# levs57/halo2-liam-eagen-msm

Hardware: AMD Instinct MI355X
Metric: BN254 G1 MSM scalar-point-pairs/s (higher is better)
Workload: dtype u32 limbs (256-bit Montgomery integers)

## Files before the change

### halo2_liam_eagen_msm_amd/api.py

```python
from __future__ import annotations

import ctypes
import math
from typing import List, Optional, Sequence, Tuple

import numpy as np

from . import _lib
from ._lib import BN254_G1, GRUMPKIN

ORDER = {
    BN254_G1: 0x30644E72E131A029B85045B68181585D2833E84879B9709143E1F593F0000001,
    GRUMPKIN: 0x30644E72E131A029B85045B68181585D97816A916871CA8D3C208C16D87CFD47,
}
CURVE_IDS = {"bn254_g1": BN254_G1, "grumpkin": GRUMPKIN}


class LemsmError(RuntimeError):
    def __init__(self, status: int, msg: str):
        super().__init__(f"lemsm status {status}: {msg}")
        self.status = status


class LengthMismatch(LemsmError, AssertionError):
# ... 671 lines not shown
        self._check(self.lib.lemsm_device_gen_walk(self.h, _curve_id(curve), _ptr(q), n, buf.ptr))
        return buf

    def debug_montmul(self, curve, a, b) -> np.ndarray:
        a = _limbs(a, 4); b = _limbs(b, 4)
        out = np.zeros_like(a)
        self._check(self.lib.lemsm_debug_montmul(self.h, _curve_id(curve), _ptr(a), _ptr(b), _ptr(out), a.shape[0]))
        return out

    def debug_fieldop(self, curve, op: int, a, b) -> np.ndarray:
        a = _limbs(a, 4); b = _limbs(b, 4)
        out = np.zeros_like(a)
        self._check(self.lib.lemsm_debug_fieldop(self.h, _curve_id(curve), op, _ptr(a), _ptr(b), _ptr(out), a.shape[0]))
        return out

    def debug_pointop(self, curve, op: int, acc_xyzz, q) -> np.ndarray:
        acc = _limbs(acc_xyzz, 16)
        q = _limbs(q, 16 if op == 1 else 8)
        out = np.zeros_like(acc)
        self._check(self.lib.lemsm_debug_pointop(self.h, _curve_id(curve), op, _ptr(acc), _ptr(q), _ptr(out), acc.shape[0]))
        return out

    F29_OPS = ("mul", "sqr", "mul2", "mul_addhi", "sqr_addhi", "add", "sub", "neg", "cneg", "wnorm", "canon", "reduce_small",
               "mul32", "from_abi", "div32", "is_zero_mod", "limbs_zero", "hi_term", "pp_is_zero")
    X29_OPS = ("madd", "madd_abi", "add", "dbl_affine", "dbl", "scale", "unscale", "add4_mem")

    def debug_field29_raw(self, curve, op, a, b=None, c=None, d=None) -> np.ndarray:
        opi = self.F29_OPS.index(op) if isinstance(op, str) else int(op)
        a = np.ascontiguousarray(a, np.int32).reshape(-1, 9)
        ops = [a] + [np.zeros_like(a) if x is None else np.ascontiguousarray(x, np.int32).reshape(-1, 9) for x in (b, c, d)]
        if any(x.shape != a.shape for x in ops):
            raise ValueError("field29_raw operands must all be n x 9 int32")
        out = np.zeros((a.shape[0], 10), np.int32)
        self._check(self.lib.lemsm_debug_field29_raw(self.h, _curve_id(curve), opi, *[_ptr(x) for x in ops], _ptr(out), a.shape[0]))
        return out

    def debug_xyzz29_raw(self, curve, op, acc, q=None) -> np.ndarray:
        opi = self.X29_OPS.index(op) if isinstance(op, str) else int(op)
        acc = np.ascontiguousarray(acc, np.int32).reshape(-1, 37)
        q = np.zeros_like(acc) if q is None else np.ascontiguousarray(q, np.int32).reshape(-1, 37)
        if q.shape != acc.shape:
            raise ValueError("xyzz29_raw records must both be n x 37 int32")
        out = np.zeros_like(acc)
        self._check(self.lib.lemsm_debug_xyzz29_raw(self.h, _curve_id(curve), opi, _ptr(acc), _ptr(q), _ptr(out), acc.shape[0]))
        return out


# ... 387 lines not shown
```

### halo2_liam_eagen_msm_amd/csrc/field29.cuh

```cuda
#pragma once
#include <hip/hip_runtime.h>
#include <stdint.h>

namespace lemsm {

typedef int32_t i32;
typedef int64_t i64;
typedef uint32_t u32;
typedef uint64_t u64;

struct Fq29Params {
  static constexpr i32 N[9] = {0x187cfd47, 0x010460b6, 0x1c72a34f, 0x02d522d0, 0x1585d978, 0x02db40c0, 0x00a6e141, 0x0e5c2634, 0x0030644e};
  static constexpr u32 NINV = 0x04866389u;
  static constexpr i32 ONE[9] = {0x157ccc21, 0x141c2758, 0x185230d3, 0x014c0419, 0x0aa36fb9, 0x1d4240ce, 0x11d54c07, 0x052ac7a8, 0x000dc836};
  static constexpr i32 C266[9] = {0x13349ca1, 0x1a5d84a8, 0x0a3e5cac, 0x100249e0, 0x12b951e8, 0x0e92d304, 0x14cb95b3, 0x041b9d3d, 0x00058003};
  static constexpr i32 C256[9] = {0x058f0d9d, 0x1aea1c6e, 0x11c2cf74, 0x11d651eb, 0x1462c0a7, 0x11b7bc3c, 0x1cbd99ba, 0x183340fb, 0x000e0a77};
};
struct Fr29Params {
  static constexpr i32 N[9] = {0x10000001, 0x1f0fac9f, 0x0e5c2450, 0x07d090f3, 0x1585d283, 0x02db40c0, 0x00a6e141, 0x0e5c2634, 0x0030644e};
  static constexpr u32 NINV = 0x0fffffffu;
  static constexpr i32 ONE[9] = {0x0fffff57, 0x1ea70ab4, 0x052c068b, 0x17504f49, 0x0aa8075b, 0x1d4240ce, 0x11d54c07, 0x052ac7a8, 0x000dc836};
  static constexpr i32 C266[9] = {0x0fffead7, 0x1d5444f4, 0x04438aa5, 0x03b4d096, 0x134c84da, 0x0e92d304, 0x14cb95b3, 0x041b9d3d, 0x00058003};
  static constexpr i32 C256[9] = {0x0ffffffb, 0x04b1a0e2, 0x18334a6b, 0x18ed2b3e, 0x1462e36f, 0x11b7bc3c, 0x1cbd99ba, 0x183340fb, 0x000e0a77};
};
// ... 11 lines not shown
  static __device__ __forceinline__ void set_one(fe& r) {
#pragma unroll
    for (int i = 0; i < 9; i++) r.l[i] = P::ONE[i];
  }
  static __device__ __forceinline__ bool limbs_zero(const fe& a) {
    i32 o = 0;
#pragma unroll
    for (int i = 0; i < 9; i++) o |= a.l[i];
    return o == 0;
  }
  static __device__ __forceinline__ void sub(fe& r, const fe& a, const fe& b) {
#pragma unroll
    for (int i = 0; i < 9; i++) r.l[i] = a.l[i] - b.l[i];
  }
  static __device__ __forceinline__ void add(fe& r, const fe& a, const fe& b) {
#pragma unroll
    for (int i = 0; i < 9; i++) r.l[i] = a.l[i] + b.l[i];
  }
  static __device__ __forceinline__ void neg(fe& r, const fe& a) {
#pragma unroll
    for (int i = 0; i < 9; i++) r.l[i] = -a.l[i];
  }
  static __device__ __forceinline__ void cneg(fe& r, const fe& a, bool flag) {
    i32 s = flag ? -1 : 0;
#pragma unroll
    for (int i = 0; i < 9; i++) r.l[i] = (a.l[i] ^ s) - s;
  }
  static __device__ __forceinline__ void wnorm(fe& a) {
    i32 c = 0;
#pragma unroll
    for (int i = 0; i < 8; i++) {
      i32 v = a.l[i] + c;
      a.l[i] = v & MASK;
      c = v >> 29;
    }
    a.l[8] += c;
  }

#include "field29_gen.inc"

  static __device__ __forceinline__ void canon(fe& a) {
    i32 c = 0;
#pragma unroll
    for (int i = 0; i < 9; i++) {
      i32 n8 = (i32)((((u32)P::N[i] << 3) & (u32)MASK) | (i ? ((u32)P::N[i - 1] >> 26) : 0u));
      i32 v = a.l[i] + n8 + c;
      if (i < 8) { a.l[i] = v & MASK; c = v >> 29; } else a.l[i] = v;
    }
#pragma unroll
// ... 45 lines not shown
    unpack(r, w);
  }
  static __device__ __forceinline__ void store(void* p, const fe& a) {
    fe t = a; canon(t);
    u32 w[8]; pack(w, t);
    uint4* q = reinterpret_cast<uint4*>(p);
    q[0] = make_uint4(w[0], w[1], w[2], w[3]);
    q[1] = make_uint4(w[4], w[5], w[6], w[7]);
  }
  static __device__ __forceinline__ void from_abi(fe& r, const fe& a) {
    fe c;
#pragma unroll
    for (int i = 0; i < 9; i++) c.l[i] = P::C266[i];
    mul(r, a, c);
  }
  static __device__ __forceinline__ void div32(fe& r, const fe& a) {
    fe c;
#pragma unroll
    for (int i = 0; i < 9; i++) c.l[i] = P::C256[i];
    mul(r, a, c);
  }
  static __device__ __forceinline__ void mul32(fe& r, const fe& a) {
    const float inv = 32.0f / (float)P::N[8];
    i32 q = (i32)((float)a.l[8] * inv);
    i64 t = 0;
#pragma unroll
    for (int i = 0; i < 9; i++) {
      t += (i64)a.l[i] * 32 - (i64)q * P::N[i];
      if (i < 8) { r.l[i] = (i32)t & MASK; t >>= 29; }
      else r.l[i] = (i32)t;
    }
  }
  static __device__ __forceinline__ void reduce_small(fe& r, const fe& a) {
    const float inv = 1.0f / (float)P::N[8];
    i32 q = (i32)((float)a.l[8] * inv);
    i64 t = 0;
#pragma unroll
    for (int i = 0; i < 9; i++) {
      t += (i64)a.l[i] - (i64)q * P::N[i];
      if (i < 8) { r.l[i] = (i32)t & MASK; t >>= 29; }
      else r.l[i] = (i32)t;
    }
  }
  static __device__ __forceinline__ void set_c266(fe& r) {
#pragma unroll
    for (int i = 0; i < 9; i++) r.l[i] = P::C266[i];
  }
};

}
```

### halo2_liam_eagen_msm_amd/csrc/field29_gen.inc

```
  static __device__ __forceinline__ void mul(fe& r, const fe& a, const fe& b) {
    i64 acc = 0;
    i32 m0, m1, m2, m3, m4, m5, m6, m7, m8;
    acc += (i64)a.l[0] * (i64)b.l[0];
    m0 = (i32)(((u32)acc * P::NINV) & (u32)MASK);
    acc += (i64)m0 * (i64)P::N[0];
    acc >>= 29;
    asm("v_mad_i64_i32 %0, vcc, %1, %2, %0\n\t"
        "v_mad_i64_i32 %0, vcc, %3, %4, %0\n\t"
        "v_mad_i64_i32 %0, vcc, %5, %6, %0\n\t" : "+v"(acc) : "v"(a.l[0]), "v"(b.l[1]), "v"(a.l[1]), "v"(b.l[0]), "v"(m0), "s"(P::N[1]) : "vcc");
    m1 = (i32)(((u32)acc * P::NINV) & (u32)MASK);
    acc += (i64)m1 * (i64)P::N[0];
    acc >>= 29;
    asm("v_mad_i64_i32 %0, vcc, %1, %2, %0\n\t"
        "v_mad_i64_i32 %0, vcc, %3, %4, %0\n\t"
        "v_mad_i64_i32 %0, vcc, %5, %6, %0\n\t"
        "v_mad_i64_i32 %0, vcc, %7, %8, %0\n\t"
        "v_mad_i64_i32 %0, vcc, %9, %10, %0\n\t" : "+v"(acc) : "v"(a.l[0]), "v"(b.l[2]), "v"(a.l[1]), "v"(b.l[1]), "v"(a.l[2]), "v"(b.l[0]), "v"(m0), "s"(P::N[2]), "v"(m1), "s"(P::N[1]) : "vcc");
    m2 = (i32)(((u32)acc * P::NINV) & (u32)MASK);
    acc += (i64)m2 * (i64)P::N[0];
    acc >>= 29;
    asm("v_mad_i64_i32 %0, vcc, %1, %2, %0\n\t"
        "v_mad_i64_i32 %0, vcc, %3, %4, %0\n\t"
        "v_mad_i64_i32 %0, vcc, %5, %6, %0\n\t"
        "v_mad_i64_i32 %0, vcc, %7, %8, %0\n\t"
// ... 986 lines not shown
    acc >>= 29;
    asm("v_mad_i64_i32 %0, vcc, %1, %2, %0\n\t"
        "v_mad_i64_i32 %0, vcc, %3, %4, %0\n\t"
        "v_mad_i64_i32 %0, vcc, %5, %6, %0\n\t"
        "v_mad_i64_i32 %0, vcc, %7, %8, %0\n\t"
        "v_mad_i64_i32 %0, vcc, %9, %10, %0\n\t" : "+v"(acc) : "v"(a2_6), "v"(a.l[8]), "v"(a.l[7]), "v"(a.l[7]), "v"(m6), "s"(P::N[8]), "v"(m7), "s"(P::N[7]), "v"(m8), "s"(P::N[6]) : "vcc");
    acc += (i64)hi.l[5];
    r.l[5] = (i32)((u32)acc & (u32)MASK);
    acc >>= 29;
    asm("v_mad_i64_i32 %0, vcc, %1, %2, %0\n\t"
        "v_mad_i64_i32 %0, vcc, %3, %4, %0\n\t"
        "v_mad_i64_i32 %0, vcc, %5, %6, %0\n\t" : "+v"(acc) : "v"(a2_7), "v"(a.l[8]), "v"(m7), "s"(P::N[8]), "v"(m8), "s"(P::N[7]) : "vcc");
    acc += (i64)hi.l[6];
    r.l[6] = (i32)((u32)acc & (u32)MASK);
    acc >>= 29;
    asm("v_mad_i64_i32 %0, vcc, %1, %2, %0\n\t"
        "v_mad_i64_i32 %0, vcc, %3, %4, %0\n\t" : "+v"(acc) : "v"(a.l[8]), "v"(a.l[8]), "v"(m8), "s"(P::N[8]) : "vcc");
    acc += (i64)hi.l[7];
    r.l[7] = (i32)((u32)acc & (u32)MASK);
    acc >>= 29;
    acc += (i64)hi.l[8];
    r.l[8] = (i32)acc;
  }
```

### halo2_liam_eagen_msm_amd/csrc/kernels_ec.cuh

```cuda
#pragma once
#include "plan.h"
#include "xyzz.cuh"
#include "xyzz29.cuh"

namespace lemsm {

static const u32 KEY_NONE = 0xffffffffu;

enum { META_M = 0, META_TILES = 1, META_WORDS = 4, META_CLOCK = 8  };

template <class G, int WPS ,
          bool ABI = false ,
          bool RING = false >
__global__ __launch_bounds__(256, WPS) void k_accum1(GroupPlan pl, const u32* __restrict__ sorted,
                                                const u32* __restrict__ bucket_start, u32* __restrict__ meta,
                                                const uint4* __restrict__ points, char* __restrict__ bucket_sum,
                                                u32* __restrict__ rec_key, char* __restrict__ rec_pt) {
  typedef typename G::F_ F;
  typedef typename F::fe fe;
  const u32 t = blockIdx.x * 256 + threadIdx.x;
  if (t >= pl.nthr1) return;
  const u32 M = meta[META_M];
  const bool stamp = blockIdx.x == (gridDim.x >> 1) && threadIdx.x == 0;
  if (stamp) {
// ... 31 lines not shown
  };

  __shared__ u32 ering[RING ? 4 : 1][2][4][64][RING ? 4 : 1];
  const u32 wv = threadIdx.x >> 6, lane = threadIdx.x & 63u;
  auto ring_fill = [&](u32 blk) {
#pragma unroll
    for (int k = 0; k < 4; k++)
      __builtin_amdgcn_global_load_lds((const __attribute__((address_space(1))) void*)(sorted + start + 16u * blk + 4u * k),
                                       (__attribute__((address_space(3))) void*)&ering[wv][blk & 1u][k][0][0], 16, 0, 0);
  };
  auto ring_read = [&](u32 rel) -> u32 { return ering[wv][(rel >> 4) & 1u][(rel >> 2) & 3u][lane][rel & 3u]; };
  u32 e_next;
  if constexpr (RING) {
    ring_fill(0);
    if (pl.L1 > 16) ring_fill(1);
    asm volatile("s_waitcnt vmcnt(0)" ::: "memory");
    e_next = ring_read(0);
  } else {
    e_next = sorted[start];
  }
  uint4 nx0, nx1, ny0, ny1;
  { const uint4* p = points + (size_t)(e_next & 0xffffffu) * 4; nx0 = p[0]; nx1 = p[1]; ny0 = p[2]; ny1 = p[3]; }

  for (u32 i = start; i < end; i++) {
    u32 e = e_next; fe px, py;
    F::from_words(px, nx0, nx1); F::from_words(py, ny0, ny1);
    if (i >= kend) {
      flush(i);
      key++; kend = kend2; kend2 = kend3;
      while (i >= kend) { key++; kend = kend2; kend2 = bucket_start[min(key + 2u, nkeys)]; }
      kbeg = i; seg_begin = i;
      G::set_identity(acc); empty = true;
    }
    if (i + 1 < end) {
      if constexpr (RING) {
        const u32 rel1 = i + 1 - start;
        if ((rel1 & 15u) == 0) asm volatile("s_waitcnt vmcnt(0)" ::: "memory");
        e_next = ring_read(rel1);
        if ((rel1 & 15u) == 0 && rel1 + 16u < pl.L1) ring_fill((rel1 >> 4) + 1u);
      } else {
        e_next = sorted[i + 1];
      }
      const uint4* p = points + (size_t)(e_next & 0xffffffu) * 4;
      nx0 = p[0]; nx1 = p[1]; ny0 = p[2]; ny1 = p[3];
    }
    kend3 = bucket_start[min(key + 3u, nkeys)];
    if (!G::aff_is_identity(px, py)) {
      F::cneg(py, py, (e >> 31) != 0);
      if (ABI) G::madd_abi(acc, px, py, empty); else G::madd(acc, px, py, empty);
    }
  }
  flush(end);
  if (stamp) {
    u64* ck = reinterpret_cast<u64*>(meta + META_CLOCK);
    ck[2] = __builtin_amdgcn_s_memtime(); ck[3] = __builtin_amdgcn_s_memrealtime();
  }
  rec_key[t] = (seg_begin == kbeg && end != kend) ? key : KEY_NONE;
}

enum { MQ_S = 0, MQ_M = 1, MQ_L = 2, MQ_F = 3, MQ_P = 4, MQ_WORDS = 16  };
static const u32 MQ_DST_BUCKET = 0xffffffffu;

template <class G>
__device__ __forceinline__ void merge_load_piece(typename G::pt& q, const char* __restrict__ rec_pt, u32 t, bool first_slot, u32 scaled) {
  G::load(q, rec_pt + (size_t)(2u * t + (first_slot ? 0u : 1u)) * G::PT_BYTES);
// ... 344 lines not shown
```

### halo2_liam_eagen_msm_amd/csrc/lemsm.hip

```cpp
#include <hip/hip_runtime.h>
#include <math.h>
#include <stdio.h>
#include <stdlib.h>
#include <string.h>

#include <algorithm>
#include <cmath>
#include <map>
#include <string>
#include <vector>

#include "../../include/lemsm.h"
#include "hostmath.hpp"
#include "hostpool.hpp"
#include "hosttail.hpp"
#include <memory>
#include "kernels.cuh"
#include "rccl_dyn.hpp"
#include "roctx_dyn.hpp"
#include "divisor.cuh"
#include "regfn_eval.cuh"
#include "regfn_logderiv.cuh"
#include "rhs.cuh"
#include <rocprim/rocprim.hpp>
// ... 1352 lines not shown
  raw_ld<F29>(x, a + 9 * (size_t)i); raw_ld<F29>(y, b + 9 * (size_t)i); raw_ld<F29>(z, c + 9 * (size_t)i); raw_ld<F29>(w, d + 9 * (size_t)i);
  int32_t pred = 0;
  r = x;
  switch (op) {
    case 0: F29::mul(r, x, y); break;
    case 1: F29::sqr(r, x); break;
    case 2: F29::mul2(r, x, y, z, w); break;
    case 3: F29::mul_addhi(r, x, y, z); break;
    case 4: F29::sqr_addhi(r, x, z); break;
    case 5: F29::add(r, x, y); break;
    case 6: F29::sub(r, x, y); break;
    case 7: F29::neg(r, x); break;
    case 8: F29::cneg(r, x, y.l[0] != 0); break;
    case 9: F29::wnorm(r); break;
    case 10: F29::canon(r); break;
    case 11: F29::reduce_small(r, x); break;
    case 12: F29::mul32(r, x); break;
    case 13: F29::from_abi(r, x); break;
    case 14: F29::div32(r, x); break;
    case 15: pred = F29::is_zero_mod(x) ? 1 : 0; break;
    case 16: pred = F29::limbs_zero(x) ? 1 : 0; break;
    case 17: G29::hi_term(r, x, y); break;
    case 18: pred = G29::pp_is_zero(x) ? 1 : 0; break;
    default: break;
  }
  int32_t* o = out + 10 * (size_t)i;
  raw_st<F29>(o, r);
  o[9] = pred;
}

template <class G29>
__device__ __forceinline__ void raw_ld_pt(typename G29::pt& p, const int32_t* s) {
  typedef typename G29::F_ F29;
  raw_ld<F29>(p.x, s); raw_ld<F29>(p.y, s + 9); raw_ld<F29>(p.zz, s + 18); raw_ld<F29>(p.zzz, s + 27);
}
template <class G29>
__device__ __forceinline__ void raw_st_pt(int32_t* s, const typename G29::pt& p) {
  typedef typename G29::F_ F29;
  raw_st<F29>(s, p.x); raw_st<F29>(s + 9, p.y); raw_st<F29>(s + 18, p.zz); raw_st<F29>(s + 27, p.zzz);
}
template <class G29>
__global__ void k_dbg_xyzz29_raw(int op, const int32_t* __restrict__ acc_in, const int32_t* __restrict__ q_in, int32_t* __restrict__ out, u32 n) {
  u32 i = blockIdx.x * blockDim.x + threadIdx.x;
  if (i >= n) return;
  const int32_t* ap = acc_in + (size_t)i * 37;
  const int32_t* qp = q_in + (size_t)i * 37;
// ... 933 lines not shown
  int rc = check_curve(ctx, curve); if (rc) return rc;
  if (!n) return LEMSM_OK;
  HIPCHK(ctx, hipSetDevice(ctx->device));
  if (op < 0 || op > 2) return fail(ctx, LEMSM_ERR_BAD_ARG, "point op: 0 madd, 1 add, 2 madd_abi");
  size_t qb = op == 1 ? 128 : 64;
  char *da, *db, *dout;
  rc = dbg_run3(ctx, acc, n * 128, q, n * qb, n * 128, &da, &db, &dout); if (rc) return rc;
  dim3 g((u32)((n + 63) / 64)), blk(64);
  if (ctx->opt_field == 0) {
    if (curve == LEMSM_BN254_G1) hipLaunchKernelGGL((k_dbg_pointop29<GqLazy>), g, blk, 0, ctx->stream, op, da, db, dout, (u32)n);
    else hipLaunchKernelGGL((k_dbg_pointop29<GrLazy>), g, blk, 0, ctx->stream, op, da, db, dout, (u32)n);
  } else if (curve == LEMSM_BN254_G1) hipLaunchKernelGGL((k_dbg_pointop<FqDev>), g, blk, 0, ctx->stream, op == 2 ? 0 : op, da, db, dout, (u32)n);
  else hipLaunchKernelGGL((k_dbg_pointop<FrDev>), g, blk, 0, ctx->stream, op == 2 ? 0 : op, da, db, dout, (u32)n);
  HIPCHK(ctx, hipGetLastError());
  HIPCHK(ctx, hipMemcpyAsync(out, dout, n * 128, hipMemcpyDeviceToHost, ctx->stream));
  HIPCHK(ctx, hipStreamSynchronize(ctx->stream));
  return LEMSM_OK;
}

int lemsm_debug_field29_raw(lemsm_ctx* ctx, int curve, int op, const int32_t* a, const int32_t* b, const int32_t* c, const int32_t* d,
                            int32_t* out, size_t n) {
  if (!ctx || !a || !b || !c || !d || !out) return LEMSM_ERR_BAD_ARG;
  int rc = check_curve(ctx, curve); if (rc) return rc;
  if (op < 0 || op > LEMSM_F29_PP_IS_ZERO) return fail(ctx, LEMSM_ERR_BAD_ARG, "field29 raw op out of range (lemsm.h LEMSM_F29_*)");
  if (!n) return LEMSM_OK;
  if (n > ((size_t)1 << 24)) return fail(ctx, LEMSM_ERR_BAD_ARG, "field29 raw: at most 2^24 operands per call");
  HIPCHK(ctx, hipSetDevice(ctx->device));
  const size_t eb = n * 36, ob = n * 40;
  size_t o1 = align_up(eb, 256), o2 = o1 + align_up(eb, 256), o3 = o2 + align_up(eb, 256), o4 = o3 + align_up(eb, 256);
  rc = reserve(ctx, ctx->ws, o4 + ob + 256); if (rc) return rc;
  char* base = (char*)ctx->ws.p;
  HIPCHK(ctx, hipMemcpyAsync(base, a, eb, hipMemcpyHostToDevice, ctx->stream));
  HIPCHK(ctx, hipMemcpyAsync(base + o1, b, eb, hipMemcpyHostToDevice, ctx->stream));
  HIPCHK(ctx, hipMemcpyAsync(base + o2, c, eb, hipMemcpyHostToDevice, ctx->stream));
  HIPCHK(ctx, hipMemcpyAsync(base + o3, d, eb, hipMemcpyHostToDevice, ctx->stream));
  const int32_t *da = (const int32_t*)base, *db = (const int32_t*)(base + o1), *dc = (const int32_t*)(base + o2), *dd = (const int32_t*)(base + o3);
  int32_t* dout = (int32_t*)(base + o4);
  dim3 g((u32)((n + 255) / 256)), blk(256);
  if (curve == LEMSM_BN254_G1) hipLaunchKernelGGL((k_dbg_field29_raw<GqLazy>), g, blk, 0, ctx->stream, op, da, db, dc, dd, dout, (u32)n);
  else hipLaunchKernelGGL((k_dbg_field29_raw<GrLazy>), g, blk, 0, ctx->stream, op, da, db, dc, dd, dout, (u32)n);
  HIPCHK(ctx, hipGetLastError());
  HIPCHK(ctx, hipMemcpyAsync(out, dout, ob, hipMemcpyDeviceToHost, ctx->stream));
  HIPCHK(ctx, hipStreamSynchronize(ctx->stream));
  return LEMSM_OK;
}

int lemsm_debug_xyzz29_raw(lemsm_ctx* ctx, int curve, int op, const int32_t* acc, const int32_t* q, int32_t* out, size_t n) {
// ... 35 lines not shown
```

### halo2_liam_eagen_msm_amd/csrc/xyzz29.cuh

```cuda
#pragma once
#include "field29.cuh"

namespace lemsm {

template <class F>
struct XYZZ29 {
  typedef F F_;
  typedef typename F::fe fe;
  static constexpr bool CONVERTED_DOMAIN = true;
  static __device__ __forceinline__ bool aff_is_identity(const fe&, const fe& y) { return F::limbs_zero(y); }
  struct pt { fe x, y, zz, zzz; };

  static __device__ __forceinline__ void set_identity(pt& p) {
    F::set_zero(p.x); F::set_zero(p.y); F::set_zero(p.zz); F::set_zero(p.zzz);
  }
  static __device__ __forceinline__ bool is_identity(const pt& p) { return F::limbs_zero(p.zz); }

  static __device__ __forceinline__ void hi_term(fe& t, const fe& ppp, const fe& q) {
#pragma unroll
    for (int i = 0; i < 9; i++) {
      i32 n2 = (i32)((((u32)F::P_::N[i] << 1) & (u32)F::MASK) | (i ? ((u32)F::P_::N[i - 1] >> 28) : 0u));
      t.l[i] = n2 - ppp.l[i] - 2 * q.l[i];
    }
  }

  static __device__ __forceinline__ bool pp_is_zero(const fe& pp) {
    if (pp.l[0] != 0 && pp.l[0] != F::P_::N[0]) return false;
    i32 z = 0, e = 0;
#pragma unroll
    for (int i = 0; i < 9; i++) { z |= pp.l[i]; e |= pp.l[i] ^ F::P_::N[i]; }
    return z == 0 || e == 0;
  }

  template <bool AFFINE>
  static __device__ __noinline__ void dbl_impl(pt& r, const pt& p) {
    fe U, V, W, S, M, t, nW, x3;
    F::add(U, p.y, p.y); F::wnorm(U);
    F::sqr(V, U);
    F::mul(W, U, V);
    F::mul(S, p.x, V);
    F::sqr(t, p.x); F::add(M, t, t); F::add(M, M, t); F::wnorm(M);
    fe zero; F::set_zero(zero);
    hi_term(t, zero, S);
    F::sqr_addhi(x3, M, t);
    F::sub(t, S, x3); F::neg(nW, W);
    fe y = p.y; F::wnorm(y);
    F::mul2(r.y, M, t, nW, y);
    r.x = x3;
    if (AFFINE) { r.zz = V; r.zzz = W; }
    else { F::mul(r.zz, V, p.zz); F::mul(r.zzz, W, p.zzz); }
  }

  static __device__ __forceinline__ void madd(pt& acc, const fe& x2, const fe& y2, bool& empty) {
    if (empty) {
      acc.x = x2; acc.y = y2; F::wnorm(acc.y); F::set_one(acc.zz); F::set_one(acc.zzz);
      empty = false;
      return;
    }
    madd_nonempty(acc, x2, y2, empty);
  }
  static __device__ __forceinline__ void madd(pt& acc, const fe& x2, const fe& y2) {
    bool empty = is_identity(acc);
    madd(acc, x2, y2, empty);
  }
  static __device__ __forceinline__ void madd_nonempty(pt& acc, const fe& x2, const fe& y2, bool& empty) {
    fe U2, S2, P, R, PP;
    F::mul(U2, x2, acc.zz);
    F::mul(S2, y2, acc.zzz);
    F::sub(P, U2, acc.x);
    F::sub(R, S2, acc.y);
    F::sqr(PP, P);
    if (pp_is_zero(PP)) {
      if (F::is_zero_mod(R)) {
        pt a, res; a.x = x2; a.y = y2; F::set_one(a.zz); F::set_one(a.zzz);
        dbl_impl<true>(res, a);
        acc = res;
      } else { set_identity(acc); empty = true; }
      return;
    }
    fe PPP, Q, t, nY;
    F::mul(PPP, P, PP);
    F::mul(Q, acc.x, PP);
    hi_term(t, PPP, Q);
    F::neg(nY, acc.y);
    F::sqr_addhi(acc.x, R, t);
    F::sub(t, Q, acc.x);
    F::mul2(acc.y, R, t, nY, PPP);
    F::mul(acc.zz, acc.zz, PP);
    F::mul(acc.zzz, acc.zzz, PPP);
  }

  static __device__ __forceinline__ void madd_abi(pt& acc, const fe& x2a, const fe& y2a, bool& empty) {
    if (empty) {
      F::mul32(acc.x, x2a); F::mul32(acc.y, y2a); F::set_c266(acc.zz); F::set_c266(acc.zzz);
      empty = false;
      return;
    }
    fe U2, S2, P, R, PP;
    F::mul(U2, x2a, acc.zz);
    F::mul(S2, y2a, acc.zzz);
    F::sub(P, U2, acc.x);
    F::sub(R, S2, acc.y);
    F::sqr(PP, P);
    if (pp_is_zero(PP)) {
      if (F::is_zero_mod(R)) {
        pt a, res; F::from_abi(a.x, x2a); F::from_abi(a.y, y2a); F::set_one(a.zz); F::set_one(a.zzz);
        dbl_impl<true>(res, a);
        F::from_abi(res.zz, res.zz); F::from_abi(res.zzz, res.zzz);
        acc = res;
      } else { set_identity(acc); empty = true; }
      return;
    }
    fe PPP, Q, t, nY;
    F::mul(PPP, P, PP);
    F::mul(Q, acc.x, PP);
    hi_term(t, PPP, Q);
    F::neg(nY, acc.y);
    F::sqr_addhi(acc.x, R, t);
    F::sub(t, Q, acc.x);
    F::mul2(acc.y, R, t, nY, PPP);
    F::mul(acc.zz, acc.zz, PP);
    F::mul(acc.zzz, acc.zzz, PPP);
  }
  static __device__ __forceinline__ void unscale(pt& p) {
    if (is_identity(p)) return;
    F::div32(p.zz, p.zz); F::div32(p.zzz, p.zzz);
  }
  static __device__ __forceinline__ void scale(pt& p) {
    if (is_identity(p)) return;
    F::from_abi(p.zz, p.zz); F::from_abi(p.zzz, p.zzz);
  }

  static __device__ __forceinline__ void add(pt& acc, const pt& q) {
    if (is_identity(q)) return;
    if (is_identity(acc)) { acc = q; return; }
    fe U1, U2, S1, S2, P, R, PP;
    F::mul(U1, acc.x, q.zz);
    F::mul(U2, q.x, acc.zz);
    F::mul(S1, acc.y, q.zzz);
    F::mul(S2, q.y, acc.zzz);
    F::sub(P, U2, U1);
    F::sub(R, S2, S1);
    F::sqr(PP, P);
    if (pp_is_zero(PP)) {
      if (F::is_zero_mod(R)) { pt t = acc, res; dbl_impl<false>(res, t); acc = res; }
      else set_identity(acc);
      return;
    }
    fe PPP, Q, t, nS;
    F::mul(PPP, P, PP);
    F::mul(Q, U1, PP);
    hi_term(t, PPP, Q);
    F::neg(nS, S1);
    F::sqr_addhi(acc.x, R, t);
    F::sub(t, Q, acc.x);
    F::mul2(acc.y, R, t, nS, PPP);
    F::mul(t, acc.zz, q.zz); F::mul(acc.zz, t, PP);
    F::mul(t, acc.zzz, q.zzz); F::mul(acc.zzz, t, PPP);
  }

  template <int CTRL>
  static __device__ __forceinline__ void quad_move(fe& r, const fe& a) {
#pragma unroll
    for (int i = 0; i < 9; i++) r.l[i] = (i32)__builtin_amdgcn_update_dpp(0, (int)a.l[i], CTRL, 0xf, 0xf, false);
  }
  static __device__ __forceinline__ void ld_elem(fe& r, const char* p, u32 k) {
    const i32* e = reinterpret_cast<const i32*>(p + 36u * k);
#pragma unroll
    for (int i = 0; i < 9; i++) r.l[i] = e[i];
  }
  static __device__ __forceinline__ void st_elem(char* p, u32 k, const fe& a) {
    i32* e = reinterpret_cast<i32*>(p + 36u * k);
#pragma unroll
    for (int i = 0; i < 9; i++) e[i] = a.l[i];
  }
  static __device__ __forceinline__ void sel(fe& r, bool c, const fe& a, const fe& b) {
#pragma unroll
// ... 99 lines not shown
```

### include/lemsm.h

```cpp
#ifndef LEMSM_H
#define LEMSM_H

#include <stddef.h>
#include <stdint.h>

#ifdef __cplusplus
extern "C" {
#endif

typedef struct lemsm_ctx lemsm_ctx;

enum lemsm_curve { LEMSM_BN254_G1 = 0, LEMSM_GRUMPKIN = 1 };

enum lemsm_status {
  LEMSM_OK = 0,
  LEMSM_ERR_LEN_MISMATCH = 1,
  LEMSM_ERR_SCALAR_OUT_OF_RANGE = 2,
  LEMSM_ERR_BAD_BASE = 3,
  LEMSM_ERR_BAD_CURVE = 4,
  LEMSM_ERR_HIP = 5,
  LEMSM_ERR_BAD_ARG = 6,
  LEMSM_ERR_NOMEM = 7,
  LEMSM_ERR_TOO_MANY_DIGITS = 8,
  LEMSM_ERR_RCCL = 9,
// ... 183 lines not shown
int lemsm_debug_montmul(lemsm_ctx* ctx, int curve, const uint64_t* a, const uint64_t* b, uint64_t* out, size_t n);
int lemsm_debug_fieldop(lemsm_ctx* ctx, int curve, int op, const uint64_t* a, const uint64_t* b, uint64_t* out, size_t n);
int lemsm_debug_pointop(lemsm_ctx* ctx, int curve, int op, const uint64_t* acc_xyzz, const uint64_t* q,
                        uint64_t* out_xyzz, size_t n);
enum {
  LEMSM_F29_MUL = 0,
  LEMSM_F29_SQR = 1,
  LEMSM_F29_MUL2 = 2,
  LEMSM_F29_MUL_ADDHI = 3,
  LEMSM_F29_SQR_ADDHI = 4,
  LEMSM_F29_ADD = 5,
  LEMSM_F29_SUB = 6,
  LEMSM_F29_NEG = 7,
  LEMSM_F29_CNEG = 8,
  LEMSM_F29_WNORM = 9,
  LEMSM_F29_CANON = 10,
  LEMSM_F29_REDUCE_SMALL = 11,
  LEMSM_F29_MUL32 = 12,
  LEMSM_F29_FROM_ABI = 13,
  LEMSM_F29_DIV32 = 14,
  LEMSM_F29_IS_ZERO_MOD = 15,
  LEMSM_F29_LIMBS_ZERO = 16,
  LEMSM_F29_HI_TERM = 17,
  LEMSM_F29_PP_IS_ZERO = 18
};
int lemsm_debug_field29_raw(lemsm_ctx* ctx, int curve, int op, const int32_t* a, const int32_t* b, const int32_t* c,
                            const int32_t* d, int32_t* out, size_t n);
enum {
  LEMSM_X29_MADD = 0,
  LEMSM_X29_MADD_ABI = 1,
  LEMSM_X29_ADD = 2,
  LEMSM_X29_DBL_AFFINE = 3,
  LEMSM_X29_DBL = 4,
  LEMSM_X29_SCALE = 5,
  LEMSM_X29_UNSCALE = 6,
  LEMSM_X29_ADD4_MEM = 7
};
int lemsm_debug_xyzz29_raw(lemsm_ctx* ctx, int curve, int op, const int32_t* acc, const int32_t* q, int32_t* out, size_t n);
int lemsm_debug_ntt(lemsm_ctx* ctx, const uint64_t* in, uint64_t* out, size_t nseq, uint32_t logn, int inverse);
int lemsm_debug_msm_sharded_sim(lemsm_ctx* ctx, int curve, const void* d_scalars, const void* d_points_affine, size_t n,
                                int world, uint64_t out_jacobian[12]);
int lemsm_debug_lhs_sharded_sim(lemsm_ctx* ctx, int curve, const void* d_scalars, const void* d_points_affine, size_t n,
                                uint8_t base, int world, uint64_t out_carry[12], uint64_t* out_carries, size_t* bad_index);

#ifdef __cplusplus
}
#endif
// ... 2 lines not shown
```

Measured before the change: 874.6 million.

## Fuse hi_term into Montgomery square, hand-tune mul32/cneg, branchless ring prefetch

Adds a fused sqr_subhi that folds the 2N - PPP - 2Q correction term into the Montgomery square's tail accumulation using inline v_mad_i64_i32. It replaces the separate hi_term plus sqr_addhi in the point add, madd and double paths. mul32 now uses mad instructions with a negated quotient, and cneg uses xor-plus-add. The ring bucket loop is made branchless on the next-element prefetch, which issues a redundant reload on the last iteration. The aim is fewer VALU instructions per EC op, at the cost of inline asm that blocks compiler scheduling.

```diff
diff --git a/halo2_liam_eagen_msm_amd/api.py b/halo2_liam_eagen_msm_amd/api.py
--- a/halo2_liam_eagen_msm_amd/api.py
+++ b/halo2_liam_eagen_msm_amd/api.py
@@ -717,7 +717,7 @@
         return out
 
     F29_OPS = ("mul", "sqr", "mul2", "mul_addhi", "sqr_addhi", "add", "sub", "neg", "cneg", "wnorm", "canon", "reduce_small",
-               "mul32", "from_abi", "div32", "is_zero_mod", "limbs_zero", "hi_term", "pp_is_zero")
+               "mul32", "from_abi", "div32", "is_zero_mod", "limbs_zero", "hi_term", "pp_is_zero", "sqr_subhi")
     X29_OPS = ("madd", "madd_abi", "add", "dbl_affine", "dbl", "scale", "unscale", "add4_mem")
 
     def debug_field29_raw(self, curve, op, a, b=None, c=None, d=None) -> np.ndarray:
diff --git a/halo2_liam_eagen_msm_amd/csrc/field29.cuh b/halo2_liam_eagen_msm_amd/csrc/field29.cuh
--- a/halo2_liam_eagen_msm_amd/csrc/field29.cuh
+++ b/halo2_liam_eagen_msm_amd/csrc/field29.cuh
@@ -57,9 +57,10 @@
     for (int i = 0; i < 9; i++) r.l[i] = -a.l[i];
   }
   static __device__ __forceinline__ void cneg(fe& r, const fe& a, bool flag) {
-    i32 s = flag ? -1 : 0;
+    const i32 s = flag ? -1 : 0;
+    const i32 t = flag ? 1 : 0;
 #pragma unroll
-    for (int i = 0; i < 9; i++) r.l[i] = (a.l[i] ^ s) - s;
+    for (int i = 0; i < 9; i++) r.l[i] = (a.l[i] ^ s) + t;
   }
   static __device__ __forceinline__ void wnorm(fe& a) {
     i32 c = 0;
@@ -151,11 +152,12 @@
   }
   static __device__ __forceinline__ void mul32(fe& r, const fe& a) {
     const float inv = 32.0f / (float)P::N[8];
-    i32 q = (i32)((float)a.l[8] * inv);
+    const i32 nq = -(i32)((float)a.l[8] * inv);
     i64 t = 0;
 #pragma unroll
     for (int i = 0; i < 9; i++) {
-      t += (i64)a.l[i] * 32 - (i64)q * P::N[i];
+      asm("v_mad_i64_i32 %0, vcc, %1, 32, %0\n\t"
+          "v_mad_i64_i32 %0, vcc, %2, %3, %0\n\t" : "+v"(t) : "v"(a.l[i]), "v"(nq), "s"(P::N[i]) : "vcc");
       if (i < 8) { r.l[i] = (i32)t & MASK; t >>= 29; }
       else r.l[i] = (i32)t;
     }
diff --git a/halo2_liam_eagen_msm_amd/csrc/field29_gen.inc b/halo2_liam_eagen_msm_amd/csrc/field29_gen.inc
--- a/halo2_liam_eagen_msm_amd/csrc/field29_gen.inc
+++ b/halo2_liam_eagen_msm_amd/csrc/field29_gen.inc
@@ -1032,3 +1032,186 @@
     acc += (i64)hi.l[8];
     r.l[8] = (i32)acc;
   }
+  static __device__ __forceinline__ void sqr_subhi(fe& r, const fe& a, const fe& ppp, const fe& q) {
+    i64 acc = 0;
+    i32 m0, m1, m2, m3, m4, m5, m6, m7, m8;
+    const i32 h0 = (i32)((((u32)P::N[0] << 1) & (u32)MASK)) - (ppp.l[0] + 2 * q.l[0]);
+    const i32 h1 = (i32)((((u32)P::N[1] << 1) & (u32)MASK) | ((u32)P::N[0] >> 28)) - (ppp.l[1] + 2 * q.l[1]);
+    const i32 h2 = (i32)((((u32)P::N[2] << 1) & (u32)MASK) | ((u32)P::N[1] >> 28)) - (ppp.l[2] + 2 * q.l[2]);
+    const i32 h3 = (i32)((((u32)P::N[3] << 1) & (u32)MASK) | ((u32)P::N[2] >> 28)) - (ppp.l[3] + 2 * q.l[3]);
+    const i32 h4 = (i32)((((u32)P::N[4] << 1) & (u32)MASK) | ((u32)P::N[3] >> 28)) - (ppp.l[4] + 2 * q.l[4]);
+    const i32 h5 = (i32)((((u32)P::N[5] << 1) & (u32)MASK) | ((u32)P::N[4] >> 28)) - (ppp.l[5] + 2 * q.l[5]);
+    const i32 h6 = (i32)((((u32)P::N[6] << 1) & (u32)MASK) | ((u32)P::N[5] >> 28)) - (ppp.l[6] + 2 * q.l[6]);
+    const i32 h7 = (i32)((((u32)P::N[7] << 1) & (u32)MASK) | ((u32)P::N[6] >> 28)) - (ppp.l[7] + 2 * q.l[7]);
+    const i32 h8 = (i32)((((u32)P::N[8] << 1) & (u32)MASK) | ((u32)P::N[7] >> 28)) - (ppp.l[8] + 2 * q.l[8]);
+    i32 a2_0 = a.l[0] * 2, a2_1 = a.l[1] * 2, a2_2 = a.l[2] * 2, a2_3 = a.l[3] * 2, a2_4 = a.l[4] * 2, a2_5 = a.l[5] * 2, a2_6 = a.l[6] * 2, a2_7 = a.l[7] * 2;
+    acc += (i64)a.l[0] * (i64)a.l[0];
+    m0 = (i32)(((u32)acc * P::NINV) & (u32)MASK);
+    acc += (i64)m0 * (i64)P::N[0];
+    acc >>= 29;
+    asm("v_mad_i64_i32 %0, vcc, %1, %2, %0\n\t"
+        "v_mad_i64_i32 %0, vcc, %3, %4, %0\n\t" : "+v"(acc) : "v"(a2_0), "v"(a.l[1]), "v"(m0), "s"(P::N[1]) : "vcc");
+    m1 = (i32)(((u32)acc * P::NINV) & (u32)MASK);
+    acc += (i64)m1 * (i64)P::N[0];
+    acc >>= 29;
+    asm("v_mad_i64_i32 %0, vcc, %1, %2, %0\n\t"
+        "v_mad_i64_i32 %0, vcc, %3, %4, %0\n\t"
+        "v_mad_i64_i32 %0, vcc, %5, %6, %0\n\t"
+        "v_mad_i64_i32 %0, vcc, %7, %8, %0\n\t" : "+v"(acc) : "v"(a2_0), "v"(a.l[2]), "v"(a.l[1]), "v"(a.l[1]), "v"(m0), "s"(P::N[2]), "v"(m1), "s"(P::N[1]) : "vcc");
+    m2 = (i32)(((u32)acc * P::NINV) & (u32)MASK);
+    acc += (i64)m2 * (i64)P::N[0];
+    acc >>= 29;
+    asm("v_mad_i64_i32 %0, vcc, %1, %2, %0\n\t"
+        "v_mad_i64_i32 %0, vcc, %3, %4, %0\n\t"
+        "v_mad_i64_i32 %0, vcc, %5, %6, %0\n\t"
+        "v_mad_i64_i32 %0, vcc, %7, %8, %0\n\t"
+        "v_mad_i64_i32 %0, vcc, %9, %10, %0\n\t" : "+v"(acc) : "v"(a2_0), "v"(a.l[3]), "v"(a2_1), "v"(a.l[2]), "v"(m0), "s"(P::N[3]), "v"(m1), "s"(P::N[2]), "v"(m2), "s"(P::N[1]) : "vcc");
+    m3 = (i32)(((u32)acc * P::NINV) & (u32)MASK);
+    acc += (i64)m3 * (i64)P::N[0];
+    acc >>= 29;
+    asm("v_mad_i64_i32 %0, vcc, %1, %2, %0\n\t"
+        "v_mad_i64_i32 %0, vcc, %3, %4, %0\n\t"
+        "v_mad_i64_i32 %0, vcc, %5, %6, %0\n\t"
+        "v_mad_i64_i32 %0, vcc, %7, %8, %0\n\t"
+        "v_mad_i64_i32 %0, vcc, %9, %10, %0\n\t"
+        "v_mad_i64_i32 %0, vcc, %11, %12, %0\n\t"
+        "v_mad_i64_i32 %0, vcc, %13, %14, %0\n\t" : "+v"(acc) : "v"(a2_0), "v"(a.l[4]), "v"(a2_1), "v"(a.l[3]), "v"(a.l[2]), "v"(a.l[2]), "v"(m0), "s"(P::N[4]), "v"(m1), "s"(P::N[3]), "v"(m2), "s"(P::N[2]), "v"(m3), "s"(P::N[1]) : "vcc");
+    m4 = (i32)(((u32)acc * P::NINV) & (u32)MASK);
+    acc += (i64)m4 * (i64)P::N[0];
+    acc >>= 29;
+    asm("v_mad_i64_i32 %0, vcc, %1, %2, %0\n\t"
+        "v_mad_i64_i32 %0, vcc, %3, %4, %0\n\t"
+        "v_mad_i64_i32 %0, vcc, %5, %6, %0\n\t"
+        "v_mad_i64_i32 %0, vcc, %7, %8, %0\n\t"
+        "v_mad_i64_i32 %0, vcc, %9, %10, %0\n\t"
+        "v_mad_i64_i32 %0, vcc, %11, %12, %0\n\t"
+        "v_mad_i64_i32 %0, vcc, %13, %14, %0\n\t"
+        "v_mad_i64_i32 %0, vcc, %15, %16, %0\n\t" : "+v"(acc) : "v"(a2_0), "v"(a.l[5]), "v"(a2_1), "v"(a.l[4]), "v"(a2_2), "v"(a.l[3]), "v"(m0), "s"(P::N[5]), "v"(m1), "s"(P::N[4]), "v"(m2), "s"(P::N[3]), "v"(m3), "s"(P::N[2]), "v"(m4), "s"(P::N[1]) : "vcc");
+    m5 = (i32)(((u32)acc * P::NINV) & (u32)MASK);
+    acc += (i64)m5 * (i64)P::N[0];
+    acc >>= 29;
+    asm("v_mad_i64_i32 %0, vcc, %1, %2, %0\n\t"
+        "v_mad_i64_i32 %0, vcc, %3, %4, %0\n\t"
+        "v_mad_i64_i32 %0, vcc, %5, %6, %0\n\t"
+        "v_mad_i64_i32 %0, vcc, %7, %8, %0\n\t"
+        "v_mad_i64_i32 %0, vcc, %9, %10, %0\n\t"
+        "v_mad_i64_i32 %0, vcc, %11, %12, %0\n\t"
+        "v_mad_i64_i32 %0, vcc, %13, %14, %0\n\t"
+        "v_mad_i64_i32 %0, vcc, %15, %16, %0\n\t"
+        "v_mad_i64_i32 %0, vcc, %17, %18, %0\n\t"
+        "v_mad_i64_i32 %0, vcc, %19, %20, %0\n\t" : "+v"(acc) : "v"(a2_0), "v"(a.l[6]), "v"(a2_1), "v"(a.l[5]), "v"(a2_2), "v"(a.l[4]), "v"(a.l[3]), "v"(a.l[3]), "v"(m0), "s"(P::N[6]), "v"(m1), "s"(P::N[5]), "v"(m2), "s"(P::N[4]), "v"(m3), "s"(P::N[3]), "v"(m4), "s"(P::N[2]), "v"(m5), "s"(P::N[1]) : "vcc");
+    m6 = (i32)(((u32)acc * P::NINV) & (u32)MASK);
+    acc += (i64)m6 * (i64)P::N[0];
+    acc >>= 29;
+    asm("v_mad_i64_i32 %0, vcc, %1, %2, %0\n\t"
+        "v_mad_i64_i32 %0, vcc, %3, %4, %0\n\t"
+        "v_mad_i64_i32 %0, vcc, %5, %6, %0\n\t"
+        "v_mad_i64_i32 %0, vcc, %7, %8, %0\n\t"
+        "v_mad_i64_i32 %0, vcc, %9, %10, %0\n\t"
+        "v_mad_i64_i32 %0, vcc, %11, %12, %0\n\t"
+        "v_mad_i64_i32 %0, vcc, %13, %14, %0\n\t"
+        "v_mad_i64_i32 %0, vcc, %15, %16, %0\n\t"
+        "v_mad_i64_i32 %0, vcc, %17, %18, %0\n\t"
+        "v_mad_i64_i32 %0, vcc, %19, %20, %0\n\t"
+        "v_mad_i64_i32 %0, vcc, %21, %22, %0\n\t" : "+v"(acc) : "v"(a2_0), "v"(a.l[7]), "v"(a2_1), "v"(a.l[6]), "v"(a2_2), "v"(a.l[5]), "v"(a2_3), "v"(a.l[4]), "v"(m0), "s"(P::N[7]), "v"(m1), "s"(P::N[6]), "v"(m2), "s"(P::N[5]), "v"(m3), "s"(P::N[4]), "v"(m4), "s"(P::N[3]), "v"(m5), "s"(P::N[2]), "v"(m6), "s"(P::N[1]) : "vcc");
+    m7 = (i32)(((u32)acc * P::NINV) & (u32)MASK);
+    acc += (i64)m7 * (i64)P::N[0];
+    acc >>= 29;
+    asm("v_mad_i64_i32 %0, vcc, %1, %2, %0\n\t"
+        "v_mad_i64_i32 %0, vcc, %3, %4, %0\n\t"
+        "v_mad_i64_i32 %0, vcc, %5, %6, %0\n\t"
+        "v_mad_i64_i32 %0, vcc, %7, %8, %0\n\t"
+        "v_mad_i64_i32 %0, vcc, %9, %10, %0\n\t"
+        "v_mad_i64_i32 %0, vcc, %11, %12, %0\n\t"
+        "v_mad_i64_i32 %0, vcc, %13, %14, %0\n\t"
+        "v_mad_i64_i32 %0, vcc, %15, %16, %0\n\t"
+        "v_mad_i64_i32 %0, vcc, %17, %18, %0\n\t"
+        "v_mad_i64_i32 %0, vcc, %19, %20, %0\n\t"
+        "v_mad_i64_i32 %0, vcc, %21, %22, %0\n\t"
+        "v_mad_i64_i32 %0, vcc, %23, %24, %0\n\t"
+        "v_mad_i64_i32 %0, vcc, %25, %26, %0\n\t" : "+v"(acc) : "v"(a2_0), "v"(a.l[8]), "v"(a2_1), "v"(a.l[7]), "v"(a2_2), "v"(a.l[6]), "v"(a2_3), "v"(a.l[5]), "v"(a.l[4]), "v"(a.l[4]), "v"(m0), "s"(P::N[8]), "v"(m1), "s"(P::N[7]), "v"(m2), "s"(P::N[6]), "v"(m3), "s"(P::N[5]), "v"(m4), "s"(P::N[4]), "v"(m5), "s"(P::N[3]), "v"(m6), "s"(P::N[2]), "v"(m7), "s"(P::N[1]) : "vcc");
+    m8 = (i32)(((u32)acc * P::NINV) & (u32)MASK);
+    acc += (i64)m8 * (i64)P::N[0];
+    acc >>= 29;
+    asm("v_mad_i64_i32 %0, vcc, %1, %2, %0\n\t"
+        "v_mad_i64_i32 %0, vcc, %3, %4, %0\n\t"
+        "v_mad_i64_i32 %0, vcc, %5, %6, %0\n\t"
+        "v_mad_i64_i32 %0, vcc, %7, %8, %0\n\t"
+        "v_mad_i64_i32 %0, vcc, %9, %10, %0\n\t"
+        "v_mad_i64_i32 %0, vcc, %11, %12, %0\n\t"
+        "v_mad_i64_i32 %0, vcc, %13, %14, %0\n\t"
+        "v_mad_i64_i32 %0, vcc, %15, %16, %0\n\t"
+        "v_mad_i64_i32 %0, vcc, %17, %18, %0\n\t"
+        "v_mad_i64_i32 %0, vcc, %19, %20, %0\n\t"
+        "v_mad_i64_i32 %0, vcc, %21, %22, %0\n\t"
+        "v_mad_i64_i32 %0, vcc, %23, %24, %0\n\t"
+        "v_mad_i64_i32 %0, vcc, %25, 1, %0\n\t" : "+v"(acc) : "v"(a2_1), "v"(a.l[8]), "v"(a2_2), "v"(a.l[7]), "v"(a2_3), "v"(a.l[6]), "v"(a2_4), "v"(a.l[5]), "v"(m1), "s"(P::N[8]), "v"(m2), "s"(P::N[7]), "v"(m3), "s"(P::N[6]), "v"(m4), "s"(P::N[5]), "v"(m5), "s"(P::N[4]), "v"(m6), "s"(P::N[3]), "v"(m7), "s"(P::N[2]), "v"(m8), "s"(P::N[1]), "v"(h0) : "vcc");
+    r.l[0] = (i32)((u32)acc & (u32)MASK);
+    acc >>= 29;
+    asm("v_mad_i64_i32 %0, vcc, %1, %2, %0\n\t"
+        "v_mad_i64_i32 %0, vcc, %3, %4, %0\n\t"
+        "v_mad_i64_i32 %0, vcc, %5, %6, %0\n\t"
+        "v_mad_i64_i32 %0, vcc, %7, %8, %0\n\t"
+        "v_mad_i64_i32 %0, vcc, %9, %10, %0\n\t"
+        "v_mad_i64_i32 %0, vcc, %11, %12, %0\n\t"
+        "v_mad_i64_i32 %0, vcc, %13, %14, %0\n\t"
+        "v_mad_i64_i32 %0, vcc, %15, %16, %0\n\t"
+        "v_mad_i64_i32 %0, vcc, %17, %18, %0\n\t"
+        "v_mad_i64_i32 %0, vcc, %19, %20, %0\n\t"
+        "v_mad_i64_i32 %0, vcc, %21, %22, %0\n\t"
+        "v_mad_i64_i32 %0, vcc, %23, 1, %0\n\t" : "+v"(acc) : "v"(a2_2), "v"(a.l[8]), "v"(a2_3), "v"(a.l[7]), "v"(a2_4), "v"(a.l[6]), "v"(a.l[5]), "v"(a.l[5]), "v"(m2), "s"(P::N[8]), "v"(m3), "s"(P::N[7]), "v"(m4), "s"(P::N[6]), "v"(m5), "s"(P::N[5]), "v"(m6), "s"(P::N[4]), "v"(m7), "s"(P::N[3]), "v"(m8), "s"(P::N[2]), "v"(h1) : "vcc");
+    r.l[1] = (i32)((u32)acc & (u32)MASK);
+    acc >>= 29;
+    asm("v_mad_i64_i32 %0, vcc, %1, %2, %0\n\t"
+        "v_mad_i64_i32 %0, vcc, %3, %4, %0\n\t"
+        "v_mad_i64_i32 %0, vcc, %5, %6, %0\n\t"
+        "v_mad_i64_i32 %0, vcc, %7, %8, %0\n\t"
+        "v_mad_i64_i32 %0, vcc, %9, %10, %0\n\t"
+        "v_mad_i64_i32 %0, vcc, %11, %12, %0\n\t"
+        "v_mad_i64_i32 %0, vcc, %13, %14, %0\n\t"
+        "v_mad_i64_i32 %0, vcc, %15, %16, %0\n\t"
+        "v_mad_i64_i32 %0, vcc, %17, %18, %0\n\t"
+        "v_mad_i64_i32 %0, vcc, %19, 1, %0\n\t" : "+v"(acc) : "v"(a2_3), "v"(a.l[8]), "v"(a2_4), "v"(a.l[7]), "v"(a2_5), "v"(a.l[6]), "v"(m3), "s"(P::N[8]), "v"(m4), "s"(P::N[7]), "v"(m5), "s"(P::N[6]), "v"(m6), "s"(P::N[5]), "v"(m7), "s"(P::N[4]), "v"(m8), "s"(P::N[3]), "v"(h2) : "vcc");
+    r.l[2] = (i32)((u32)acc & (u32)MASK);
+    acc >>= 29;
+    asm("v_mad_i64_i32 %0, vcc, %1, %2, %0\n\t"
+        "v_mad_i64_i32 %0, vcc, %3, %4, %0\n\t"
+        "v_mad_i64_i32 %0, vcc, %5, %6, %0\n\t"
+        "v_mad_i64_i32 %0, vcc, %7, %8, %0\n\t"
+        "v_mad_i64_i32 %0, vcc, %9, %10, %0\n\t"
+        "v_mad_i64_i32 %0, vcc, %11, %12, %0\n\t"
+        "v_mad_i64_i32 %0, vcc, %13, %14, %0\n\t"
+        "v_mad_i64_i32 %0, vcc, %15, %16, %0\n\t"
+        "v_mad_i64_i32 %0, vcc, %17, 1, %0\n\t" : "+v"(acc) : "v"(a2_4), "v"(a.l[8]), "v"(a2_5), "v"(a.l[7]), "v"(a.l[6]), "v"(a.l[6]), "v"(m4), "s"(P::N[8]), "v"(m5), "s"(P::N[7]), "v"(m6), "s"(P::N[6]), "v"(m7), "s"(P::N[5]), "v"(m8), "s"(P::N[4]), "v"(h3) : "vcc");
+    r.l[3] = (i32)((u32)acc & (u32)MASK);
+    acc >>= 29;
+    asm("v_mad_i64_i32 %0, vcc, %1, %2, %0\n\t"
+        "v_mad_i64_i32 %0, vcc, %3, %4, %0\n\t"
+        "v_mad_i64_i32 %0, vcc, %5, %6, %0\n\t"
+        "v_mad_i64_i32 %0, vcc, %7, %8, %0\n\t"
+        "v_mad_i64_i32 %0, vcc, %9, %10, %0\n\t"
+        "v_mad_i64_i32 %0, vcc, %11, %12, %0\n\t"
+        "v_mad_i64_i32 %0, vcc, %13, 1, %0\n\t" : "+v"(acc) : "v"(a2_5), "v"(a.l[8]), "v"(a2_6), "v"(a.l[7]), "v"(m5), "s"(P::N[8]), "v"(m6), "s"(P::N[7]), "v"(m7), "s"(P::N[6]), "v"(m8), "s"(P::N[5]), "v"(h4) : "vcc");
+    r.l[4] = (i32)((u32)acc & (u32)MASK);
+    acc >>= 29;
+    asm("v_mad_i64_i32 %0, vcc, %1, %2, %0\n\t"
+        "v_mad_i64_i32 %0, vcc, %3, %4, %0\n\t"
+        "v_mad_i64_i32 %0, vcc, %5, %6, %0\n\t"
+        "v_mad_i64_i32 %0, vcc, %7, %8, %0\n\t"
+        "v_mad_i64_i32 %0, vcc, %9, %10, %0\n\t"
+        "v_mad_i64_i32 %0, vcc, %11, 1, %0\n\t" : "+v"(acc) : "v"(a2_6), "v"(a.l[8]), "v"(a.l[7]), "v"(a.l[7]), "v"(m6), "s"(P::N[8]), "v"(m7), "s"(P::N[7]), "v"(m8), "s"(P::N[6]), "v"(h5) : "vcc");
+    r.l[5] = (i32)((u32)acc & (u32)MASK);
+    acc >>= 29;
+    asm("v_mad_i64_i32 %0, vcc, %1, %2, %0\n\t"
+        "v_mad_i64_i32 %0, vcc, %3, %4, %0\n\t"
+        "v_mad_i64_i32 %0, vcc, %5, %6, %0\n\t"
+        "v_mad_i64_i32 %0, vcc, %7, 1, %0\n\t" : "+v"(acc) : "v"(a2_7), "v"(a.l[8]), "v"(m7), "s"(P::N[8]), "v"(m8), "s"(P::N[7]), "v"(h6) : "vcc");
+    r.l[6] = (i32)((u32)acc & (u32)MASK);
+    acc >>= 29;
+    asm("v_mad_i64_i32 %0, vcc, %1, %2, %0\n\t"
+        "v_mad_i64_i32 %0, vcc, %3, %4, %0\n\t"
+        "v_mad_i64_i32 %0, vcc, %5, 1, %0\n\t" : "+v"(acc) : "v"(a.l[8]), "v"(a.l[8]), "v"(m8), "s"(P::N[8]), "v"(h7) : "vcc");
+    r.l[7] = (i32)((u32)acc & (u32)MASK);
+    acc >>= 29;
+    r.l[8] = (i32)acc + h8;
+  }
diff --git a/halo2_liam_eagen_msm_amd/csrc/kernels_ec.cuh b/halo2_liam_eagen_msm_amd/csrc/kernels_ec.cuh
--- a/halo2_liam_eagen_msm_amd/csrc/kernels_ec.cuh
+++ b/halo2_liam_eagen_msm_amd/csrc/kernels_ec.cuh
@@ -77,7 +77,8 @@
   uint4 nx0, nx1, ny0, ny1;
   { const uint4* p = points + (size_t)(e_next & 0xffffffu) * 4; nx0 = p[0]; nx1 = p[1]; ny0 = p[2]; ny1 = p[3]; }
 
-  for (u32 i = start; i < end; i++) {
+  u32 rel = 0;
+  for (u32 i = start; i < end; i++, rel++) {
     u32 e = e_next; fe px, py;
     F::from_words(px, nx0, nx1); F::from_words(py, ny0, ny1);
     if (i >= kend) {
@@ -87,15 +88,18 @@
       kbeg = i; seg_begin = i;
       G::set_identity(acc); empty = true;
     }
-    if (i + 1 < end) {
-      if constexpr (RING) {
-        const u32 rel1 = i + 1 - start;
-        if ((rel1 & 15u) == 0) asm volatile("s_waitcnt vmcnt(0)" ::: "memory");
-        e_next = ring_read(rel1);
-        if ((rel1 & 15u) == 0 && rel1 + 16u < pl.L1) ring_fill((rel1 >> 4) + 1u);
-      } else {
-        e_next = sorted[i + 1];
-      }
+    if constexpr (RING) {
+      const bool more = i + 1 < end;
+      const u32 rel1 = rel + 1;
+      const bool turn = (rel1 & 15u) == 0;
+      if (turn) asm volatile("s_waitcnt vmcnt(0)" ::: "memory");
+      const u32 en = ring_read(rel1);
+      e_next = more ? en : e;
+      if (turn && rel1 + 16u < pl.L1) { if (more) ring_fill((rel1 >> 4) + 1u); }
+      const uint4* p = points + (size_t)(e_next & 0xffffffu) * 4;
+      nx0 = p[0]; nx1 = p[1]; ny0 = p[2]; ny1 = p[3];
+    } else if (i + 1 < end) {
+      e_next = sorted[i + 1];
       const uint4* p = points + (size_t)(e_next & 0xffffffu) * 4;
       nx0 = p[0]; nx1 = p[1]; ny0 = p[2]; ny1 = p[3];
     }
diff --git a/halo2_liam_eagen_msm_amd/csrc/lemsm.hip b/halo2_liam_eagen_msm_amd/csrc/lemsm.hip
--- a/halo2_liam_eagen_msm_amd/csrc/lemsm.hip
+++ b/halo2_liam_eagen_msm_amd/csrc/lemsm.hip
@@ -1398,6 +1398,7 @@
     case 16: pred = F29::limbs_zero(x) ? 1 : 0; break;
     case 17: G29::hi_term(r, x, y); break;
     case 18: pred = G29::pp_is_zero(x) ? 1 : 0; break;
+    case 19: F29::sqr_subhi(r, x, y, z); break;
     default: break;
   }
   int32_t* o = out + 10 * (size_t)i;
@@ -2377,7 +2378,7 @@
                             int32_t* out, size_t n) {
   if (!ctx || !a || !b || !c || !d || !out) return LEMSM_ERR_BAD_ARG;
   int rc = check_curve(ctx, curve); if (rc) return rc;
-  if (op < 0 || op > LEMSM_F29_PP_IS_ZERO) return fail(ctx, LEMSM_ERR_BAD_ARG, "field29 raw op out of range (lemsm.h LEMSM_F29_*)");
+  if (op < 0 || op > LEMSM_F29_SQR_SUBHI) return fail(ctx, LEMSM_ERR_BAD_ARG, "field29 raw op out of range (lemsm.h LEMSM_F29_*)");
   if (!n) return LEMSM_OK;
   if (n > ((size_t)1 << 24)) return fail(ctx, LEMSM_ERR_BAD_ARG, "field29 raw: at most 2^24 operands per call");
   HIPCHK(ctx, hipSetDevice(ctx->device));
diff --git a/halo2_liam_eagen_msm_amd/csrc/xyzz29.cuh b/halo2_liam_eagen_msm_amd/csrc/xyzz29.cuh
--- a/halo2_liam_eagen_msm_amd/csrc/xyzz29.cuh
+++ b/halo2_liam_eagen_msm_amd/csrc/xyzz29.cuh
@@ -41,8 +41,7 @@
     F::mul(S, p.x, V);
     F::sqr(t, p.x); F::add(M, t, t); F::add(M, M, t); F::wnorm(M);
     fe zero; F::set_zero(zero);
-    hi_term(t, zero, S);
-    F::sqr_addhi(x3, M, t);
+    F::sqr_subhi(x3, M, zero, S);
     F::sub(t, S, x3); F::neg(nW, W);
     fe y = p.y; F::wnorm(y);
     F::mul2(r.y, M, t, nW, y);
@@ -81,9 +80,8 @@
     fe PPP, Q, t, nY;
     F::mul(PPP, P, PP);
     F::mul(Q, acc.x, PP);
-    hi_term(t, PPP, Q);
     F::neg(nY, acc.y);
-    F::sqr_addhi(acc.x, R, t);
+    F::sqr_subhi(acc.x, R, PPP, Q);
     F::sub(t, Q, acc.x);
     F::mul2(acc.y, R, t, nY, PPP);
     F::mul(acc.zz, acc.zz, PP);
@@ -114,9 +112,8 @@
     fe PPP, Q, t, nY;
     F::mul(PPP, P, PP);
     F::mul(Q, acc.x, PP);
-    hi_term(t, PPP, Q);
     F::neg(nY, acc.y);
-    F::sqr_addhi(acc.x, R, t);
+    F::sqr_subhi(acc.x, R, PPP, Q);
     F::sub(t, Q, acc.x);
     F::mul2(acc.y, R, t, nY, PPP);
     F::mul(acc.zz, acc.zz, PP);
@@ -150,9 +147,8 @@
     fe PPP, Q, t, nS;
     F::mul(PPP, P, PP);
     F::mul(Q, U1, PP);
-    hi_term(t, PPP, Q);
     F::neg(nS, S1);
-    F::sqr_addhi(acc.x, R, t);
+    F::sqr_subhi(acc.x, R, PPP, Q);
     F::sub(t, Q, acc.x);
     F::mul2(acc.y, R, t, nS, PPP);
     F::mul(t, acc.zz, q.zz); F::mul(acc.zz, t, PP);
diff --git a/include/lemsm.h b/include/lemsm.h
--- a/include/lemsm.h
+++ b/include/lemsm.h
@@ -229,7 +229,8 @@
   LEMSM_F29_IS_ZERO_MOD = 15,
   LEMSM_F29_LIMBS_ZERO = 16,
   LEMSM_F29_HI_TERM = 17,
-  LEMSM_F29_PP_IS_ZERO = 18
+  LEMSM_F29_PP_IS_ZERO = 18,
+  LEMSM_F29_SQR_SUBHI = 19
 };
 int lemsm_debug_field29_raw(lemsm_ctx* ctx, int curve, int op, const int32_t* a, const int32_t* b, const int32_t* c,
                             const int32_t* d, int32_t* out, size_t n);
```

New measurement: 884.0 million (median of 6 runs). +1.1%, better.
